# danini/multi-h

Measured on AMD Instinct MI355X. Metric: scored homography hypotheses/sec (50k pts x 100k models), higher is better.
Workload: dtype f64

## Files before the change

multi-h_amd/csrc/capi_engine.hpp:

```cpp
#pragma once
#include "../../include/multih_hip.h"
#include "mh_kernels.hpp"

#include <algorithm>
#include <chrono>
#include <cstdlib>
#include <cmath>
#include <cstdio>
#include <cstring>
#include <string>
#include <utility>
#include <atomic>
#include <memory>
#include <thread>
#include <vector>

using namespace mh;

extern thread_local std::string g_err;

inline int fail(int code, const std::string& msg)
{
    g_err = msg;
    return code;
// ... 168 lines not shown
    DevBuf<unsigned long long> sel_keys;
    int t_rank = 0, t_world = 1;
    mh_allgather_stream_fn t_stream_fn = nullptr;
    mh_allgather_dev_fn t_host_fn = nullptr;
    void* t_ctx = nullptr;
    Stream side_stream;
    Event ev_main, ev_side_pre;
    int tune_score32_resident = 12;
    int occ_score32 = -1, occ_cost32 = -1;
    int tune_cost32_batched = 0;
    int tune_cost32_slice_major = 0;
    int tune_sweep_slices = 0;
    int tune_dlt_variant = 0;
    int tune_cost32_resident = 8;
    int tune_stream_shift = 0;
    Stream dummy_streams[16];
    int tune_dlt_first = 1;
    static constexpr int PF_DEPTH = 2;
    DevBuf<double> pf_H[PF_DEPTH];
    DevBuf<int> pf_samples[PF_DEPTH];
    int pf_m[PF_DEPTH] = { 0, 0 };
    Event pf_ev[PF_DEPTH];
    int pf_head = 0, pf_count = 0;
    Stream xchg_stream;
    Event ev_sweep, ev_x[3];
    CountsSlot counts_waiting[2];
    long long xchg_calls = 0;
    long long models_seq = 0, best_models_seq = -1;
    bool counts_zeroed = false;
    bool counts_fresh = false;
    bool xchg_pending = false;
    PinnedBuf<int> h_best;
    int best_seq = 0;
    PinnedBuf<int> h_sel;
    long long copies_h2d = 0, copies_d2h = 0;

    int fm = 0;
    int fund_metric = 0;
    DevBuf<double> fund, fund_one;
    DevBuf<int> fund_samples, fund_counts, fund_inl;
    int fund_tuple = 8;
    int f7_m = 0;
    DevBuf<int> fund_nvalid, fund_stop;
    DevBuf<unsigned char> fund_mask, ref_keep, ref_in, ref_reason;
    int ref_reason_n = 0;
    DevBuf<double> ref_out;

    DevBuf<double> loc_H, loc_feat, ms_data, ms_mean;
    DevBuf<int> ms_votes, ms_out, ms_list, ms_pcnt, ms_heads, ms_tickets;
    DevBuf<double> ms_partial, ms_partial2;
    DevBuf<unsigned long long> ms_ticks;
    DevBuf<int> ms_ctl, ms_pcnt2;
    int ms_persist_per_cu = -1, ms_persist_per_cu6 = -1;
    int tune_select_refine = 0;
    int estimator = MH_ESTIMATOR_HAF;
    int data_term = MH_DATA_TERM_REFERENCE;
    DevBuf<int> r3_scratch;
    int tune_3pt_form = 0;
    DevBuf<double> sel_refit;
    DevBuf<int> sel_refit_ctr;
    DevBuf<double> ms_rs;
    DevBuf<int> ms_order, ms_cells, ms_cursor, ms_cellcount;
    int tune_ms_indexed = 1;
    int tune_ms_dense = 8;
    long long ms_indexed_launches = 0;
    int tune_ms_persist = 12;
    long long ms_persist_launches = 0, ms_persist_fallbacks = 0, ms_rounds = 0;

    int cost_L = 0;
    DevBuf<int> cost, labels_in, labels_pts, label_counts;
    DevBuf<int> ew_label, ew_cur, ew_trace, ew_saved, d_order, d_wsum;
    int comp_moves = 0;
    DevBuf<int> ew_comp, ew_comp_out;
    int trace_moves = 0;
    int detail_move = -1;
    ExpandCtxBufs ew_ctx[EXPAND_MAX_CTX];
    DevBuf<int> ew_bctl;
    PinnedBuf<int> h_batch;
    int tune_expand_ctx = 16;
    int tune_batch_min_labels = 16;
    int tune_batch_spw = 0;
    int cu_count = 256;
    DevBuf<int> sweep_ctl;
    int sweep_wg_per_cu = -1;
    int tune_sweep_headroom = 0;
    int solve_grid_max = 0;
    double longest_barrier_wait_ms = 0.0;
    int last_expand_retries = 0;
    long long expand_retries_total = 0;
    int last_solve_grid = 0;
    int inject_select_failure = 0;
    int inject_barrier_timeouts = 0;
    int inject_solve_failure = 0;
    PinnedBuf<int> h_flags;
    PinnedBuf<long long> h_acc;
    PinnedBuf<MeanShiftResultBlock> h_ms;
    PinnedBuf<int> h_ms_list;
    DevBuf<double> sel_pts[4];
    DevBuf<int> sel_pack_count;
    DevBuf<double> sel_gone[4];
    int tune_select_decrement = 1;
    int tune_knn_grid = 1;
    DevBuf<int> knn_cell, knn_count, knn_start, knn_orig;
    DevBuf<float> knn_P;
    DevBuf<int> knn_tmp, knn_part_i;
    DevBuf<float> knn_part_d;
    int sampler = MH_SAMPLER_UNIFORM, sampler_uniform_per_16 = 0;
    DevBuf<int> smp_nbr;
    int smp_k = 0;
    Dlt4Local dlt_local() const { return sampler == MH_SAMPLER_LOCAL ? Dlt4Local{ smp_nbr.p, smp_k, sampler_uniform_per_16 } : Dlt4Local{}; }

    bool profiling = false;
    KernelTimer timers[MH_K_COUNT_];
    int tune_residual_variant = 0;
    int tune_ld = 0;
    int tune_score_variant = 0;
    int residual_mode = MH_RESIDUAL_FORWARD;
    int tune_ms_batch = 6;
    int tune_reduce = 2;
    int tune_reduce_launches = 1;
    int tune_recycle = 1;
    int tune_expand[4] = { 128, 512, 1, 256 };
    int tune_cascade_iters = 2;
    int tune_push_mult = 6;
    ExpandStats last_expand{};

    double bbox[4] = { NAN, NAN, NAN, NAN };
    bool coords32_ok = false;
    double absmax_x = NAN, absmax_y = NAN, absmax_dst = NAN;
    int tune_score32_tiling = 0;
    int tune_score32 = 1;
    DevBuf<float> H32;
    DevBuf<unsigned long long> fb_pairs;
    long long score_pairs = 0;
    long long score_pairs_plain_fp64 = 0;
    DevBuf<int> weights, weights_counts;
    long long weights_models_seq = -1;
    PinnedBuf<int> h_best_w;
    Points pts() const { return Points{ x1.p, y1.p, x2.p, y2.p, n, bbox[0], bbox[1], bbox[2], bbox[3] }; }
};

namespace mhe {

template <typename Fn>
int guarded(Fn&& fn)
{
    try {
        return fn();
    } catch (const std::bad_alloc&) {
        return fail(MH_ERR_INVALID, "out of host memory");
    } catch (const std::exception& ex) {
        return fail(MH_ERR_INVALID, std::string("internal error: ") + ex.what());
    } catch (...) {
        return fail(MH_ERR_INVALID, "internal error");
    }
}

struct ScopedTimer {
    mh_engine* e;
    int k;
    hipStream_t st;
    Event a, b;
    bool on = false;
    ScopedTimer(mh_engine* e_, int k_, hipStream_t on_stream = nullptr) : e(e_), k(k_), st(on_stream ? on_stream : e_->stream)
    {
        if (!e->profiling || a.ensure(hipEventDefault) != hipSuccess || b.ensure(hipEventDefault) != hipSuccess) return;
        (void)hipEventRecord(a, st);
// ... 56 lines not shown
```

multi-h_amd/csrc/capi_score.hip:

```cpp
#include "capi_engine.hpp"

namespace mhe {

static bool pretest_usable(const mh_engine* e, double thr2, bool plain_variant_only)
{
    if (plain_variant_only && e->tune_score_variant != 0) return false;
    return e->tune_score32 && e->coords32_ok && thr2 >= 0x1p-40 && thr2 <= 0x1p40;
}

static int ensure_sweep_ctl(mh_engine* e)
{
    if (!e->sweep_ctl.p) {
        HIPCHK(e->sweep_ctl.reserve(2));
        HIPCHK(hipMemsetAsync(e->sweep_ctl.p, 0, sizeof(int) * 2, e->stream));
    }
    return MH_OK;
}

int score_models(mh_engine* e, const Points& p, const double* Hs, int m, double thr2, const unsigned char* dmask, int* counts_dev)
{
    const bool fwd = e->residual_mode != MH_RESIDUAL_SYMMETRIC;
    if (fwd && m > 0 && pretest_usable(e, thr2, true)) {
        HIPCHK(e->H32.reserve((size_t)m * 16));
        HIPCHK(e->fb_pairs.reserve(1));
// ... 147 lines not shown
    return guarded([&]() -> int {
    if (!e) return fail(MH_ERR_INVALID, "null engine");
    if (mode != MH_RESIDUAL_FORWARD && mode != MH_RESIDUAL_SYMMETRIC) return fail(MH_ERR_INVALID, "unknown residual mode");
    e->residual_mode = mode;
    return MH_OK;
    });
}

int mh_score(mh_engine* e, double thr2, const unsigned char* point_mask, int* counts)
{
    return guarded([&]() -> int {
    bool empty_shard = false;
    int rc = require_models_or_empty_shard(e, &empty_shard);
    if (rc || empty_shard) return rc;
    HIPCHK(reserve_counts(e, (size_t)e->m + 1));
    const unsigned char* dmask = nullptr;
    if (point_mask) {
        HIPCHK(e->mask.reserve((size_t)e->n + 2));
        HIPCHK(hipMemcpyAsync(e->mask.p, point_mask, e->n, hipMemcpyHostToDevice, e->stream));
        dmask = e->mask.p;
    }
    {
        ScopedTimer t(e, MH_K_SCORE);
        rc = score_models(e, e->pts(), e->H.p, e->m, thr2, dmask, e->counts.p);
        if (rc) return rc;
    }
    counts_scored(e);
    if (counts) {
        HIPCHK(hipMemcpyAsync(counts, e->counts.p, sizeof(int) * e->m, hipMemcpyDeviceToHost, e->stream));
        HIPCHK(hipStreamSynchronize(e->stream));
    }
    return MH_OK;
    });
}

int mh_score_msac(mh_engine* e, double thr2, const unsigned char* point_mask, int* counts, int* weights)
{
    return guarded([&]() -> int {
    bool empty_shard = false;
    int rc = require_models_or_empty_shard(e, &empty_shard);
    if (rc || empty_shard) return rc;
    if (e->residual_mode == MH_RESIDUAL_SYMMETRIC) return fail(MH_ERR_INVALID, "mh_score_msac: forward residual only");
    if ((long long)e->n * MH_MSAC_SCALE > 2147483647ll) return fail(MH_ERR_OVERFLOW, "mh_score_msac: n * MH_MSAC_SCALE exceeds int32");
    HIPCHK(reserve_counts(e, (size_t)e->m + 1));
    HIPCHK(e->weights.reserve((size_t)e->m + 1));
    HIPCHK(e->weights_counts.reserve((size_t)e->m + 1));
    const unsigned char* dmask = nullptr;
    if (point_mask) {
        HIPCHK(e->mask.reserve((size_t)e->n + 2));
        HIPCHK(hipMemcpyAsync(e->mask.p, point_mask, e->n, hipMemcpyHostToDevice, e->stream));
        dmask = e->mask.p;
    }
    e->weights_models_seq = -1;
    {
        ScopedTimer t(e, MH_K_SCORE);
        rc = msac_models(e, e->pts(), e->H.p, e->m, thr2, dmask, e->counts.p, e->weights.p, false);
        if (rc) return rc;
    }
    HIPCHK(hipMemcpyAsync(e->weights_counts.p, e->counts.p, sizeof(int) * (size_t)e->m, hipMemcpyDeviceToDevice, e->stream));
    counts_scored(e);
    e->weights_models_seq = e->models_seq;
    if (counts) HIPCHK(hipMemcpyAsync(counts, e->counts.p, sizeof(int) * e->m, hipMemcpyDeviceToHost, e->stream));
    if (weights) HIPCHK(hipMemcpyAsync(weights, e->weights.p, sizeof(int) * e->m, hipMemcpyDeviceToHost, e->stream));
    if (counts || weights) HIPCHK(hipStreamSynchronize(e->stream));
    return MH_OK;
    });
}

int mh_residual_matrix(mh_engine* e, double thr2, double* R_host, int* counts)
{
    return guarded([&]() -> int {
    bool empty_shard = false;
    int rc = require_models_or_empty_shard(e, &empty_shard);
    if (rc || empty_shard) return rc;
    e->ldr = residual_ld(e->n);
    size_t r_elems = (size_t)e->m * (size_t)e->ldr;
#ifdef MH_TUNING
    if (e->tune_ld > 0) { e->ldr = std::max<long long>(e->tune_ld, e->ldr); r_elems = (size_t)e->m * (size_t)e->ldr; }
    r_elems = std::max(r_elems, (size_t)((e->m + 15) / 16 * 16) * (size_t)((e->n + 1023) / 1024 * 1024));
#endif
    HIPCHK(e->R.reserve(r_elems));
    HIPCHK(reserve_counts(e, (size_t)e->m + 1));
    int resident = 0;
    if (e->tune_sweep_headroom >= 0 && e->residual_mode != MH_RESIDUAL_SYMMETRIC && (e->tune_residual_variant == 0 || (e->tune_residual_variant >= 50 && e->tune_residual_variant <= 52))) {
        if (e->sweep_wg_per_cu < 0) e->sweep_wg_per_cu = residual_workgroups_per_cu();
        const int headroom = e->tune_sweep_headroom > 0 ? e->tune_sweep_headroom : (e->t_stream_fn && e->t_world > 1 ? 32 : 0);
        resident = e->sweep_wg_per_cu * e->cu_count - headroom;
        if (resident < e->cu_count) resident = 0;
        if (resident > 0) {
            rc = ensure_sweep_ctl(e);
            if (rc) return rc;
        }
    }
    if (e->pf_count == 1 && e->tune_dlt_first && e->ev_side_pre) HIPCHK(hipStreamWaitEvent(e->stream, e->ev_side_pre, 0));
    {
        ScopedTimer t(e, MH_K_RESIDUAL);
        SweepLaunch how;
        how.slices = e->tune_sweep_slices;
        how.slice_major = e->tune_sweep_slices > 0 ? 1 : 0;
        how.counts_zeroed = e->counts_zeroed;
        how.resident_grid = resident;
        how.resident_ctl = e->sweep_ctl.p;
        HIPCHK(launch_residual(e->pts(), e->H.p, e->m, thr2, e->R.p, e->ldr, e->counts.p,
                               e->residual_mode == MH_RESIDUAL_SYMMETRIC ? -1 : e->tune_residual_variant, e->stream, how));
    }
    counts_scored(e);
    if (R_host)
        HIPCHK(hipMemcpy2DAsync(R_host, sizeof(double) * e->n, e->R.p, sizeof(double) * e->ldr,
                                sizeof(double) * e->n, e->m, hipMemcpyDeviceToHost, e->stream));
    if (counts)
        HIPCHK(hipMemcpyAsync(counts, e->counts.p, sizeof(int) * e->m, hipMemcpyDeviceToHost, e->stream));
    if (R_host || counts) HIPCHK(hipStreamSynchronize(e->stream));
    return MH_OK;
    });
}

int mh_cost_matrix(mh_engine* e, int* C_host, int* counts)
{
    return guarded([&]() -> int {
    bool empty_shard = false;
    int rc = require_models_or_empty_shard(e, &empty_shard);
    if (rc || empty_shard) return rc;
    e->ldc = cost_ld(e->n);
    HIPCHK(e->C.reserve((size_t)e->m * (size_t)e->ldc));
    HIPCHK(reserve_counts(e, (size_t)e->m + 1));
    {
        ScopedTimer t(e, MH_K_COSTMATRIX);
        const double thr2 = e->thr_H * e->thr_H;
        if (pretest_usable(e, thr2, false)) {
            HIPCHK(e->H32.reserve((size_t)e->m * 16));
            HIPCHK(launch_model32(e->H.p, e->m, e->absmax_x, e->absmax_y, e->absmax_dst, e->H32.p, e->stream));
            int* ctl = nullptr;
            if (e->tune_cost32_resident != 0) {
                rc = ensure_sweep_ctl(e);
                if (rc) return rc;
                ctl = e->sweep_ctl.p;
            }
            HIPCHK(launch_cost32(e->pts(), e->H.p, e->H32.p, e->m, e->lambda, thr2, e->absmax_dst, e->C.p, e->ldc, e->counts.p, e->stream,
                                 ctl, e->cu_count, e->tune_cost32_resident > 0 ? e->tune_cost32_resident : 0, e->tune_cost32_slice_major, e->tune_cost32_batched, &e->occ_cost32,
                                 e->data_term == MH_DATA_TERM_RISING));
        } else
            HIPCHK(launch_cost_matrix(e->pts(), e->H.p, e->m, e->lambda, thr2, e->C.p, e->ldc, e->counts.p, e->stream,
                                      e->data_term == MH_DATA_TERM_RISING));
    }
    counts_scored(e);
    if (C_host)
        HIPCHK(hipMemcpy2DAsync(C_host, sizeof(int) * e->n, e->C.p, sizeof(int) * e->ldc, sizeof(int) * e->n, e->m,
                                hipMemcpyDeviceToHost, e->stream));
    if (counts) HIPCHK(hipMemcpyAsync(counts, e->counts.p, sizeof(int) * e->m, hipMemcpyDeviceToHost, e->stream));
    if (C_host || counts) HIPCHK(hipStreamSynchronize(e->stream));
    return MH_OK;
    });
}

int mh_get_residual_rows(mh_engine* e, int first, int count, double* rows_host)
{
    return guarded([&]() -> int {
    int rc = require_models(e);
    if (rc) return rc;
    if (!e->R.p || e->ldr <= 0) return fail(MH_ERR_NOT_SET, "residual matrix has not been computed");
    if (first < 0 || count <= 0 || first + count > e->m || !rows_host)
        return fail(MH_ERR_INVALID, "row range out of bounds or null output");
    HIPCHK(hipMemcpy2DAsync(rows_host, sizeof(double) * e->n, e->R.p + (size_t)first * e->ldr,
                            sizeof(double) * e->ldr, sizeof(double) * e->n, count,
                            hipMemcpyDeviceToHost, e->stream));
    HIPCHK(hipStreamSynchronize(e->stream));
    return MH_OK;
    });
}

int mh_prefetch_dlt4(mh_engine* e, unsigned long long seed, long long first, int m)
{
    return guarded([&]() -> int {
    int rc = require_points(e);
    if (rc) return rc;
    if (m <= 0) return fail(MH_ERR_INVALID, "m must be positive");
    if (e->n < 4) return fail(MH_ERR_INVALID, "need at least 4 correspondences");
    if (e->sampler == MH_SAMPLER_LOCAL && e->smp_k <= 0) return fail(MH_ERR_NOT_SET, "the local sampler has no table; call mh_build_sample_neighbours");
    rc = ensure_side_stream(e);
    if (rc) return rc;
    if (e->pf_count >= mh_engine::PF_DEPTH) return fail(MH_ERR_INVALID, "two batches are already prefetched: adopt one first (mh_adopt_prefetched)");
    const int slot = (e->pf_head + e->pf_count) % mh_engine::PF_DEPTH;
    if (e->pf_H[slot].cap < (size_t)m * 9 || e->pf_samples[slot].cap < (size_t)m * 4) {
        HIPCHK(hipStreamSynchronize(e->side_stream));
        HIPCHK(hipStreamSynchronize(e->stream));
        HIPCHK(e->pf_H[slot].reserve((size_t)m * 9));
        HIPCHK(e->pf_samples[slot].reserve((size_t)m * 4));
// ... 111 lines not shown
```

multi-h_amd/csrc/mh_kernels.hpp:

```cpp
#pragma once
#include <hip/hip_runtime.h>
#include <cstdint>

namespace mh {

struct Points {
    const double* x1;
    const double* y1;
    const double* x2;
    const double* y2;
    int n;
    double xmin, xmax, ymin, ymax;
};

struct Affines {
    const double* a11;
    const double* a12;
    const double* a21;
    const double* a22;
};

struct Epipolar {
    double F[9];
    double ex, ey;
};

inline long long residual_ld(int n) { return ((long long)n + 15) & ~15ll; }

struct SweepLaunch {
    int slices = 0;
    bool contiguous = false;
    int swapxy = 0;
    bool counts_zeroed = false;
    int resident_grid = 0;
    int* resident_ctl = nullptr;
    int slice_major = 0;
};
hipError_t launch_residual(const Points& p, const double* H, int M, double thr2, double* R,
                           long long ldr, int* counts, int variant, hipStream_t s, const SweepLaunch& how);
int residual_workgroups_per_cu();
hipError_t launch_score(const Points& p, const double* H, int M, double thr2,
                        const unsigned char* mask, int* counts, int variant, hipStream_t s);
hipError_t launch_model32(const double* H, int M, double X, double Y, double Cmax, float* H32 , hipStream_t s);
hipError_t launch_score32(const Points& p, const double* H, const float* H32, int M, double thr2, double Cmax, const unsigned char* mask,
                          int* counts, unsigned long long* fallback_pairs, int tiling, hipStream_t s, int* resident_ctl = nullptr,
                          int cu_count = 256, int resident_slices = 0, int* occ_cache = nullptr);
hipError_t launch_cost32(const Points& p, const double* H, const float* H32, int M, double lambda, double thr2, double Cmax,
                         int* C, long long ldc, int* counts, hipStream_t s, int* resident_ctl = nullptr, int cu_count = 256,
                         int psplit_override = 0, int slice_major = 0, int batched = 0, int* occ_cache = nullptr, int rising = 0);
hipError_t launch_msac32(const Points& p, const double* H, const float* H32, int M, double thr2, double Cmax, const unsigned char* mask,
                         int* counts, int* weights, unsigned long long* fp64_pairs, hipStream_t s);
hipError_t launch_msac64(const Points& p, const double* H, int M, double thr2, const unsigned char* mask, int* counts, int* weights,
                         hipStream_t s);
hipError_t launch_inliers_of_model(const Points& p, const double* H, int idx, double thr2,
                                   int label_value, int* labels, hipStream_t s);
hipError_t launch_moments(const Points& p, const double* H, int M, double thr2, double* moments,
                          double* min_eig, hipStream_t s);

hipError_t launch_compat_select(const double* pts , const int* begin , int clusters,
                                const int* tri , const double* H ,
                                const unsigned char* ok, int trials, double* out , hipStream_t s);
hipError_t launch_compat_fit(const double* pts, const int* begin, int clusters, const int* tri, const double F[9], int trials,
                             double* H, unsigned char* ok, hipStream_t s);

struct Dlt4Local { const int* nbr = nullptr; int k = 0; int uniform_per_16 = 0; };
hipError_t launch_dlt4(const Points& p, unsigned long long seed, long long first, int M,
                       int* idx_out, double* H_out, hipStream_t s, int variant = 0 ,
                       Dlt4Local local = Dlt4Local{});

hipError_t launch_fund8(const Points& p, unsigned long long seed, long long first, int M,
                        int* idx_out , double* F_out, hipStream_t s);

hipError_t launch_fund7(const Points& p, unsigned long long seed, long long first, int M,
                        int* idx_out , double* F_out , int* nvalid_out , hipStream_t s);

hipError_t launch_ransac_stop(const int* counts , const int* nvalid , int S, int n, double confidence,
                              const double* F , double* F_win, int* out, hipStream_t s);
hipError_t launch_fund_mask(const Points& p, const double* F_in, double thr2, unsigned char* mask_out, int* count,
                            hipStream_t s, int metric);
hipError_t launch_sampson_score(const Points& p, const double* F, int M, double thr2, int* counts,
                                hipStream_t s, int metric);
hipError_t launch_fund_refit(const Points& p, const double* F_in, double thr2, double* F_out,
                             unsigned char* mask_out, int* count_out, hipStream_t s, int metric);

constexpr int REFIT_H_MAX_ITERATIONS = 16;
hipError_t launch_refit_h(const Points& p, const double* H_in, double thr2, int iterations, double* H_out,
                          unsigned char* mask_out, int* out_i, hipStream_t s);

inline long long cost_ld(int n) { return ((long long)n + 31) & ~31ll; }
hipError_t launch_cost_matrix(const Points& p, const double* H, int M, double lambda, double thr2, int* C, long long ldc,
                              int* counts, hipStream_t s, int rising = 0);
hipError_t launch_data_cost(const Points& p, const double* H, int Nh, double lambda, double thr2,
                            int* cost, hipStream_t s, int rising = 0);

hipError_t launch_reestimate(const Points& p, const Affines& a, const int* labels, int Nh,
                             const Epipolar& ep, double* H, int* counts, hipStream_t s);

size_t reestimate_3pt_scratch_ints(int n, int Nh);
hipError_t launch_reestimate_3pt(const Points& p, const int* labels, int Nh, const Epipolar& ep, double* H, int* counts,
                                 int* scratch, hipStream_t s, int form = 0);

hipError_t launch_haf_point(const Points& p, const Affines& a, const Epipolar& ep, double locality,
                            double* H_out , double* feat_out ,
                            hipStream_t s);

hipError_t launch_haf_propose(const Points& p, const Affines& a, const Epipolar& ep, const int* nbr, int k, int members,
                              double thr2, long long first, int m, int stride, double* H_out, unsigned* used_out, hipStream_t s);

hipError_t launch_propose_3pt(const Points& p, const double F[9], unsigned long long seed, long long first, int M,
                              int* idx_out, double* H_out, hipStream_t s, Dlt4Local local = Dlt4Local{});

hipError_t launch_refine_points(const Points& p, const Affines& a, const double F[9], const double e1[2],
                                const double e2[2], const unsigned char* in_mask, unsigned char* keep,
                                double* out , unsigned char* reason , hipStream_t s,
                                int points_only = 0);

constexpr int MS_BATCH = 256;
struct MeanShiftWork {
    const double* data;
    int n, d;
    double* mean;
    int* votes;
    int* out;
// ... 185 lines not shown
```

multi-h_amd/csrc/residual.hip:

```cpp

#include <type_traits>

#include "mh_kernels.hpp"
#include "mh_device.hpp"

namespace mh {

typedef double __attribute__((address_space(1))) gdouble;
typedef char __attribute__((address_space(1))) gchar;

namespace cfg {
struct Base {
    static constexpr bool WRITE_R = false, MASK = false, SYM = false, NT = false, FAST = true, HSGPR = false, LEAN = false, SEMI = true;
    static constexpr bool CALIB = false, CONTRACT = false, TILED = false;
    static constexpr int SF = 0, MINW = 1;
};
struct Sweep : Base { static constexpr int PPL = 4, MC = 64; static constexpr bool WRITE_R = true, NT = true, HSGPR = true, LEAN = true; };
struct SweepSym : Base { static constexpr int PPL = 4, MC = 16; static constexpr bool WRITE_R = true, NT = true, HSGPR = true, SYM = true; };
struct Score : Base { static constexpr int PPL = 4, MC = 16; static constexpr bool HSGPR = true, LEAN = true; };
struct ScoreMasked : Score { static constexpr bool MASK = true; };
struct ScoreSym : Base { static constexpr int PPL = 4, MC = 16; static constexpr bool SYM = true; };
struct ScoreSymMasked : ScoreSym { static constexpr bool MASK = true; };
template <class... C> constexpr bool no_measurement_switch = ((!C::CALIB && !C::CONTRACT && !C::TILED && C::SF == 0 && C::MINW == 1 && C::FAST && C::PPL == 4) && ...);
static_assert(no_measurement_switch<Sweep, SweepSym, Score, ScoreMasked, ScoreSym, ScoreSymMasked>, "a measurement switch in a product form");
}
using ProductSweep = cfg::Sweep;

template <class Cfg> constexpr bool on_resident_grid = false;
template <> constexpr bool on_resident_grid<ProductSweep> = true;

template <class Cfg>
__device__ __forceinline__ void
residual_wg(const double* __restrict__ x1, const double* __restrict__ y1,
            const double* __restrict__ x2, const double* __restrict__ y2, int N,
            const double* __restrict__ H, int M, double thr2, double* __restrict__ R,
            long long ldr, int* __restrict__ counts, const unsigned char* __restrict__ mask,
            int psplit, double bx0, double bx1, double by0, double by1, const int bx, const int by)
{
    constexpr int PPL = Cfg::PPL, MC = Cfg::MC, SF = Cfg::SF;
    constexpr bool WRITE_R = Cfg::WRITE_R, MASK = Cfg::MASK, NT = Cfg::NT, FAST = Cfg::FAST, CALIB = Cfg::CALIB, HSGPR = Cfg::HSGPR,
                   SYM = Cfg::SYM, CONTRACT = Cfg::CONTRACT, LEAN = Cfg::LEAN, TILED = Cfg::TILED, SEMI = Cfg::SEMI;
    constexpr int CH = PPL / 2;
    constexpr int WAVE_PTS = 64 * PPL;
    constexpr int TILE = 4 * WAVE_PTS;
    const int lane = threadIdx.x & 63;
    const int wave = __builtin_amdgcn_readfirstlane(threadIdx.x >> 6);
    const int m0 = bx * MC;

    __shared__ double s_h[MC * 9];
    __shared__ double s_a[SYM ? MC * 9 : 1];
    for (int i = threadIdx.x; i < MC * 9; i += 256) {
        const size_t g = (size_t)m0 * 9 + i;
        s_h[i] = (g < (size_t)M * 9) ? H[g] : 0.0;
    }
    __shared__ int s_hok[MC];
    __shared__ int s_far[MC];
    __shared__ int s_aok[SYM ? MC : 1];
    __syncthreads();
    if (threadIdx.x < MC) {
        const double* h = s_h + 9 * threadIdx.x;
        s_hok[threadIdx.x] = model_pre(h);
        s_far[threadIdx.x] = model_far(h, bx0, bx1, by0, by1);
        if (SYM) {
            double* a = s_a + 9 * threadIdx.x;
            a[0] = h[4] * h[8] - h[5] * h[7]; a[1] = h[2] * h[7] - h[1] * h[8]; a[2] = h[1] * h[5] - h[2] * h[4];
            a[3] = h[5] * h[6] - h[3] * h[8]; a[4] = h[0] * h[8] - h[2] * h[6]; a[5] = h[2] * h[3] - h[0] * h[5];
            a[6] = h[3] * h[7] - h[4] * h[6]; a[7] = h[1] * h[6] - h[0] * h[7]; a[8] = h[0] * h[4] - h[1] * h[3];
            s_aok[threadIdx.x] = model_pre(a);
        }
    }
    __syncthreads();

    const unsigned long long hok_bits = __builtin_amdgcn_ballot_w64(lane < MC && s_hok[lane < MC ? lane : 0] != 0);
    const unsigned long long far_bits = __builtin_amdgcn_ballot_w64(lane < MC && s_far[lane < MC ? lane : 0] != 0);

    unsigned lane_bytes = (unsigned)lane * 16u;

    int cnt = 0;
    static_assert(MC <= 64, "one counting lane per model");

    const int nslices = psplit > 0 ? psplit : -psplit;
    const int ntiles_all = (N + TILE - 1) / TILE;
    const int per_slice = (ntiles_all + nslices - 1) / nslices;
    const int base0 = psplit > 0 ? by * TILE : by * per_slice * TILE;
    const int base_end = psplit > 0 ? N : min(N, (by + 1) * per_slice * TILE);
    const int base_step = psplit > 0 ? psplit * TILE : TILE;
    for (int base = base0; base < base_end; base += base_step) {
        double px[PPL], py[PPL], qx[PPL], qy[PPL];
        bool ok[PPL], pok[PPL], pokb[SYM ? PPL : 1];
        unsigned long long okm[PPL];
        const int wbase = base + wave * WAVE_PTS;
#pragma unroll
        for (int c = 0; c < CH; ++c) {
            const int n = wbase + c * 128 + lane * 2;
            if (n + 1 < N) {
                const double2 a = *reinterpret_cast<const double2*>(x1 + n);
                const double2 b = *reinterpret_cast<const double2*>(y1 + n);
                const double2 cc = *reinterpret_cast<const double2*>(x2 + n);
                const double2 d = *reinterpret_cast<const double2*>(y2 + n);
                px[2 * c] = a.x; px[2 * c + 1] = a.y;
                py[2 * c] = b.x; py[2 * c + 1] = b.y;
                qx[2 * c] = cc.x; qx[2 * c + 1] = cc.y;
                qy[2 * c] = d.x; qy[2 * c + 1] = d.y;
                ok[2 * c] = true; ok[2 * c + 1] = true;
            } else if (n < N) {
                px[2 * c] = x1[n]; py[2 * c] = y1[n]; qx[2 * c] = x2[n]; qy[2 * c] = y2[n];
                px[2 * c + 1] = 1.0; py[2 * c + 1] = 1.0; qx[2 * c + 1] = 1.0; qy[2 * c + 1] = 1.0;
                ok[2 * c] = true; ok[2 * c + 1] = false;
            } else {
                px[2 * c] = 1.0; py[2 * c] = 1.0; qx[2 * c] = 1.0; qy[2 * c] = 1.0;
                px[2 * c + 1] = 1.0; py[2 * c + 1] = 1.0; qx[2 * c + 1] = 1.0; qy[2 * c + 1] = 1.0;
                ok[2 * c] = false; ok[2 * c + 1] = false;
            }
            if (MASK) {
                if (ok[2 * c]) ok[2 * c] = mask[n] != 0;
                if (ok[2 * c + 1]) ok[2 * c + 1] = mask[n + 1] != 0;
            }
            okm[2 * c] = __builtin_amdgcn_ballot_w64(ok[2 * c]);
            okm[2 * c + 1] = __builtin_amdgcn_ballot_w64(ok[2 * c + 1]);
            pok[2 * c] = point_pre(px[2 * c], py[2 * c], qx[2 * c], qy[2 * c]);
            pok[2 * c + 1] = point_pre(px[2 * c + 1], py[2 * c + 1], qx[2 * c + 1], qy[2 * c + 1]);
            if (SYM) {
                pokb[2 * c] = point_pre(qx[2 * c], qy[2 * c], px[2 * c], py[2 * c]);
                pokb[2 * c + 1] = point_pre(qx[2 * c + 1], qy[2 * c + 1], px[2 * c + 1], py[2 * c + 1]);
            }
        }

        bool tile_lean = false;
        if (LEAN) {
            bool lane_ok = true;
#pragma unroll
            for (int q = 0; q < PPL; ++q) lane_ok = lane_ok && ok[q] && pok[q];
            tile_lean = (wbase + WAVE_PTS <= N) && (__builtin_amdgcn_ballot_w64(lane_ok) == ~0ull);
        }
        const int tile_idx = base / TILE;

#pragma unroll 1
        for (int mi = 0; mi < MC; ++mi) {
            const int m = m0 + mi;
            if (m < M) {
                const double* h = HSGPR ? (H + 9 * (size_t)m) : (s_h + 9 * mi);
                const double h0 = h[0], h1 = h[1], h2 = h[2], h3 = h[3], h4 = h[4], h5 = h[5],
                             h6 = h[6], h7 = h[7], h8 = h[8];
                const bool hok = ((hok_bits >> mi) & 1ull) != 0;
                const bool far = FAST && !CONTRACT && ((far_bits >> mi) & 1ull) != 0;
                const bool aok = SYM ? (s_aok[mi] != 0) : false;
                int c_m = 0;
                auto row_ptr = [&](int n) -> double* {
                    if (TILED) return R + ((size_t)bx * ntiles_all + tile_idx) * ((size_t)MC * TILE) + (size_t)mi * TILE + (n - base);
                    return R + (size_t)m * ldr + n;
                };
                gchar* row_base = (gchar*)row_ptr(wbase);
                asm volatile("" : "+v"(lane_bytes));
                asm volatile("" : "+s"(row_base));
                auto sweep = [&](auto schk) {
                    constexpr bool SCHK = decltype(schk)::value;
#pragma unroll
                    for (int c = 0; c < CH; ++c) {
                        if (CALIB) {
                            const int n = wbase + c * 128 + lane * 2;
                            if (n + 1 < N)
                                *reinterpret_cast<double2*>(R + (size_t)m * ldr + n) =
                                    make_double2(px[2 * c] + h0, py[2 * c] + h0);
                            continue;
                        }
                        double d0s, d1s;
                        const double d0 = CONTRACT ? fwd_d2_contracted(h0, h1, h2, h3, h4, h5, h6, h7, h8, px[2 * c],
                                                                       py[2 * c], qx[2 * c], qy[2 * c])
                                          : FAST ? fwd_d2_fast<SCHK>(h0, h1, h2, h3, h4, h5, h6, h7, h8, px[2 * c],
                                                                   py[2 * c], qx[2 * c], qy[2 * c], pok[2 * c] && hok)
                                               : fwd_d2(h0, h1, h2, h3, h4, h5, h6, h7, h8, px[2 * c],
                                                        py[2 * c], qx[2 * c], qy[2 * c]);
                        const double d1 = CONTRACT ? fwd_d2_contracted(h0, h1, h2, h3, h4, h5, h6, h7, h8, px[2 * c + 1],
                                                                       py[2 * c + 1], qx[2 * c + 1], qy[2 * c + 1])
                                          : FAST ? fwd_d2_fast<SCHK>(h0, h1, h2, h3, h4, h5, h6, h7, h8, px[2 * c + 1],
                                                                   py[2 * c + 1], qx[2 * c + 1], qy[2 * c + 1], pok[2 * c + 1] && hok)
                                               : fwd_d2(h0, h1, h2, h3, h4, h5, h6, h7, h8, px[2 * c + 1],
                                                        py[2 * c + 1], qx[2 * c + 1], qy[2 * c + 1]);
                        d0s = d0; d1s = d1;
                        if (SYM) {
                            const double* a = s_a + 9 * mi;
                            const double b0 = fwd_d2_fast<true>(a[0], a[1], a[2], a[3], a[4], a[5], a[6], a[7], a[8],
                                                                qx[2 * c], qy[2 * c], px[2 * c], py[2 * c], pokb[2 * c] && aok);
                            const double b1 = fwd_d2_fast<true>(a[0], a[1], a[2], a[3], a[4], a[5], a[6], a[7], a[8],
                                                                qx[2 * c + 1], qy[2 * c + 1], px[2 * c + 1], py[2 * c + 1],
                                                                pokb[2 * c + 1] && aok);
                            d0s = d0 + b0;
                            d1s = d1 + b1;
                        }
                        if (WRITE_R) {
                            const int n = wbase + c * 128 + lane * 2;
                            gdouble* dstp = reinterpret_cast<gdouble*>(row_base + lane_bytes) + c * 128;
                            if (n + 1 < N) {
                                if (NT) {
                                    __builtin_nontemporal_store(d0s, dstp);
                                    __builtin_nontemporal_store(d1s, dstp + 1);
                                } else {
                                    dstp[0] = d0s; dstp[1] = d1s;
                                }
                            } else if (n < N) {
                                dstp[0] = d0s;
                            }
                        }
                        c_m += __builtin_popcountll(__builtin_amdgcn_ballot_w64(d0s < thr2) & okm[2 * c]);
                        c_m += __builtin_popcountll(__builtin_amdgcn_ballot_w64(d1s < thr2) & okm[2 * c + 1]);
                    }
                };
                bool lean_done = false;
                if (LEAN && FAST && !SYM && !CONTRACT && !CALIB && tile_lean && hok && (SEMI || far)) {
                    double dl[PPL], sq[PPL];
                    unsigned long long bad = 0ull;
#pragma unroll
                    for (int q = 0; q < PPL; ++q)
                        dl[q] = fwd_d2_lean(h0, h1, h2, h3, h4, h5, h6, h7, h8, px[q], py[q], qx[q], qy[q], sq[q]);
                    if (!far) {
#pragma unroll
                        for (int q = 0; q < PPL; ++q) bad |= __builtin_amdgcn_ballot_w64(!(__builtin_fabs(sq[q]) >= 0x1p-255));
                    }
                    if (bad == 0ull) {
                        lean_done = true;
#pragma unroll
                        for (int c = 0; c < CH; ++c) {
                            const double d0 = dl[2 * c], d1 = dl[2 * c + 1];
                            if (WRITE_R) {
                                gdouble* dstp = reinterpret_cast<gdouble*>(row_base + lane_bytes) + c * 128;
                                if (SF != 0) {
                                    typedef double d2v __attribute__((ext_vector_type(2)));
                                    const d2v val = { d0, d1 };
                                    if (SF == 2) asm volatile("global_store_dwordx4 %0, %1, off sc1" :: "v"(dstp), "v"(val) : "memory");
                                    else if (SF == 3) asm volatile("global_store_dwordx4 %0, %1, off sc0 sc1" :: "v"(dstp), "v"(val) : "memory");
                                    else if (SF == 4) asm volatile("global_store_dwordx4 %0, %1, off sc1 nt" :: "v"(dstp), "v"(val) : "memory");
                                    else asm volatile("global_store_dwordx4 %0, %1, off sc0 sc1 nt" :: "v"(dstp), "v"(val) : "memory");
                                } else if (NT) {
                                    __builtin_nontemporal_store(d0, dstp);
                                    __builtin_nontemporal_store(d1, dstp + 1);
                                } else {
                                    dstp[0] = d0; dstp[1] = d1;
                                }
                            }
                            c_m += __builtin_popcountll(__builtin_amdgcn_ballot_w64(d0 < thr2));
                            c_m += __builtin_popcountll(__builtin_amdgcn_ballot_w64(d1 < thr2));
                        }
                    }
                }
                if (lean_done) {}
                else if (far) sweep(std::false_type{});
                else sweep(std::true_type{});
                const int c_new = __builtin_amdgcn_readlane(cnt, mi) + c_m;
                asm("s_mov_b32 m0, %2\n\ts_nop 0\n\tv_writelane_b32 %0, %1, m0" : "+v"(cnt) : "s"(c_new), "s"(mi) : "m0");
            }
        }
    }

    __shared__ int s_cnt[4][MC];
    if (lane < MC) s_cnt[wave][lane] = cnt;
    __syncthreads();
    if (threadIdx.x < MC && m0 + (int)threadIdx.x < M) {
        const int t = threadIdx.x;
        const int c = s_cnt[0][t] + s_cnt[1][t] + s_cnt[2][t] + s_cnt[3][t];
        if (nslices == 1) counts[m0 + t] = c;
        else atomicAdd(&counts[m0 + t], c);
    }
}

template <class Cfg>
__global__ void __launch_bounds__(256, Cfg::MINW)
k_residual(const double* __restrict__ x1, const double* __restrict__ y1,
           const double* __restrict__ x2, const double* __restrict__ y2, int N,
           const double* __restrict__ H, int M, double thr2, double* __restrict__ R,
           long long ldr, int* __restrict__ counts, const unsigned char* __restrict__ mask,
           int psplit, int swapxy, double bx0, double bx1, double by0, double by1)
{
    const int bx = swapxy ? blockIdx.y : blockIdx.x;
    const int by = swapxy ? blockIdx.x : blockIdx.y;
    residual_wg<Cfg>(x1, y1, x2, y2, N, H, M, thr2, R, ldr, counts, mask, psplit, bx0, bx1, by0, by1, bx, by);
}

template <class Cfg>
__global__ void __launch_bounds__(256, Cfg::MINW) __attribute__((amdgpu_num_vgpr(88)))
k_residual_resident(const double* __restrict__ x1, const double* __restrict__ y1,
                    const double* __restrict__ x2, const double* __restrict__ y2, int N,
                    const double* __restrict__ H, int M, double thr2, double* __restrict__ R,
                    long long ldr, int* __restrict__ counts, const unsigned char* __restrict__ mask,
                    int psplit, int gx, int nitems, int* __restrict__ ctl, double bx0, double bx1, double by0, double by1, int slice_major)
{
    __shared__ int s_item;
#pragma unroll 1
    for (;;) {
        if (threadIdx.x == 0) s_item = atomicAdd(&ctl[0], 1);
        __syncthreads();
        const int item = s_item;
        if (item >= nitems) break;
        int bx, by;
        if (slice_major) { bx = item / psplit; by = item - bx * psplit; }
        else { by = item / gx; bx = item - by * gx; }
        residual_wg<Cfg>(x1, y1, x2, y2, N, H, M, thr2, R, ldr, counts, mask, psplit, bx0, bx1, by0, by1, bx, by);
        __syncthreads();
    }
    if (threadIdx.x == 0 && atomicAdd(&ctl[1], 1) == (int)gridDim.x - 1) {
        ctl[1] = 0;
        __hip_atomic_store(&ctl[0], 0, __ATOMIC_RELEASE, __HIP_MEMORY_SCOPE_AGENT);
    }
}

template <class Cfg>
static hipError_t launch_rs(const Points& p, const double* H, int M, double thr2, double* R,
                            long long ldr, int* counts, const unsigned char* mask, hipStream_t s, const SweepLaunch& how = {})
{
    constexpr int PPL = Cfg::PPL, MC = Cfg::MC;
    if (M <= 0 || p.n <= 0) return hipSuccess;
    const int gx = (M + MC - 1) / MC;
    const int tile = 256 * PPL;
    const int ntiles = (p.n + tile - 1) / tile;
    int psplit = 1;
    if (Cfg::WRITE_R) {
        psplit = (37500 + gx - 1) / gx;
        if (psplit < 4 && ntiles >= 32) psplit = 4;
        if (psplit > ntiles) psplit = ntiles;
        if (psplit < 1) psplit = 1;
    } else if (gx < 1024) {
        psplit = (2048 + gx - 1) / gx;
        if (psplit > ntiles) psplit = ntiles;
        if (psplit < 1) psplit = 1;
    } else if (ntiles >= 32) {
        psplit = 4;
    }
    const bool forced = how.slices > 0, contiguous = forced && how.contiguous;
    if (forced) psplit = how.slices < ntiles ? how.slices : ntiles;
    if (psplit > 1 && !how.counts_zeroed) {
        hipError_t e = hipMemsetAsync(counts, 0, sizeof(int) * (size_t)M, s);
        if (e != hipSuccess) return e;
    }
    if constexpr (on_resident_grid<Cfg>)
    if (how.resident_grid > 0 && how.resident_ctl && !contiguous && !how.swapxy && gx * psplit > how.resident_grid) {
        hipLaunchKernelGGL(k_residual_resident<Cfg>, dim3(how.resident_grid), dim3(256), 0, s, p.x1, p.y1, p.x2, p.y2, p.n, H, M, thr2, R,
                           ldr, counts, mask, psplit, gx, gx * psplit, how.resident_ctl, p.xmin, p.xmax, p.ymin, p.ymax, how.slice_major);
        return hipGetLastError();
    }
    dim3 grid(gx, psplit);
    if (how.swapxy) grid = dim3(psplit, gx);
    hipLaunchKernelGGL(k_residual<Cfg>, grid, dim3(256), 0, s, p.x1, p.y1, p.x2, p.y2, p.n, H, M, thr2, R, ldr, counts, mask,
                       contiguous ? -psplit : psplit, how.swapxy, p.xmin, p.xmax, p.ymin, p.ymax);
    return hipGetLastError();
}

#ifdef MH_TUNING
namespace tune {
static hipError_t launch_residual_variant(const Points& p, const double* H, int M, double thr2, double* R, long long ldr, int* counts,
                                          int variant, hipStream_t s, const SweepLaunch& how);
static hipError_t launch_score_variant(const Points& p, const double* H, int M, double thr2, int* counts, int variant, hipStream_t s);
}
#endif

hipError_t launch_residual(const Points& p, const double* H, int M, double thr2, double* R,
                           long long ldr, int* counts, int variant, hipStream_t s, const SweepLaunch& how)
{
    auto run = [&](auto form, const SweepLaunch& o = {}) { return launch_rs<decltype(form)>(p, H, M, thr2, R, ldr, counts, nullptr, s, o); };
    if (variant == 0) return run(ProductSweep{}, how);
    if (variant == -1) return run(cfg::SweepSym{});
#ifdef MH_TUNING
    return tune::launch_residual_variant(p, H, M, thr2, R, ldr, counts, variant, s, how);
#else
    return hipErrorInvalidValue;
#endif
}

int residual_workgroups_per_cu()
{
    int n = 0;
    const hipError_t he = hipOccupancyMaxActiveBlocksPerMultiprocessor(&n, (const void*)k_residual_resident<ProductSweep>, 256, 0);
    return he == hipSuccess && n > 0 ? n : 0;
}

hipError_t launch_score(const Points& p, const double* H, int M, double thr2,
                        const unsigned char* mask, int* counts, int variant, hipStream_t s)
{
    auto run = [&](auto form) { return launch_rs<decltype(form)>(p, H, M, thr2, nullptr, 0, counts, mask, s); };
    if (variant == -1) return mask ? run(cfg::ScoreSymMasked{}) : run(cfg::ScoreSym{});
    if (mask) return run(cfg::ScoreMasked{});
    if (variant == 0) return run(cfg::Score{});
#ifdef MH_TUNING
    return tune::launch_score_variant(p, H, M, thr2, counts, variant, s);
#else
    return hipErrorInvalidValue;
#endif
}

#ifdef MH_TUNING
#include "residual_variants.hpp"
#endif

__global__ void __launch_bounds__(256)
k_inliers_of_model(const double* __restrict__ x1, const double* __restrict__ y1,
                   const double* __restrict__ x2, const double* __restrict__ y2, int N,
                   const double* __restrict__ H, int idx, double thr2, int label_value,
                   int* __restrict__ labels)
{
    const int n = blockIdx.x * 256 + threadIdx.x;
    if (n >= N) return;
    const double* h = H + 9 * (size_t)idx;
    const double d2 = fwd_d2(h[0], h[1], h[2], h[3], h[4], h[5], h[6], h[7], h[8], x1[n], y1[n],
                             x2[n], y2[n]);
    if (d2 < thr2) labels[n] = label_value;
}

hipError_t launch_inliers_of_model(const Points& p, const double* H, int idx, double thr2,
                                   int label_value, int* labels, hipStream_t s)
{
    hipLaunchKernelGGL(k_inliers_of_model, dim3((p.n + 255) / 256), dim3(256), 0, s, p.x1, p.y1,
                       p.x2, p.y2, p.n, H, idx, thr2, label_value, labels);
    return hipGetLastError();
}

__global__ void __launch_bounds__(256)
k_moments(const double* __restrict__ x1, const double* __restrict__ y1,
          const double* __restrict__ x2, const double* __restrict__ y2, int N,
          const double* __restrict__ H, double thr2, double* __restrict__ moments,
          double* __restrict__ min_eig)
{
    const int m = blockIdx.x;
    const int t = threadIdx.x;
    const double* h = H + 9 * (size_t)m;
    const double h0 = h[0], h1 = h[1], h2 = h[2], h3 = h[3], h4 = h[4], h5 = h[5], h6 = h[6],
                 h7 = h[7], h8 = h[8];
    double acc[5] = { 0.0, 0.0, 0.0, 0.0, 0.0 };
    int cnt = 0;
    constexpr int UNROLL = 8;
    for (int n0 = t; n0 < N; n0 += 256 * UNROLL) {
        double px[UNROLL], py[UNROLL], qx[UNROLL], qy[UNROLL];
#pragma unroll
        for (int j = 0; j < UNROLL; ++j) {
            const int n = n0 + 256 * j, mm = n < N ? n : 0;
            px[j] = x1[mm]; py[j] = y1[mm]; qx[j] = x2[mm]; qy[j] = y2[mm];
        }
#pragma unroll
        for (int j = 0; j < UNROLL; ++j) {
            if (n0 + 256 * j >= N) continue;
            const double x = px[j], y = py[j];
            const double d2 = fwd_d2(h0, h1, h2, h3, h4, h5, h6, h7, h8, x, y, qx[j], qy[j]);
            if (d2 < thr2) {
                acc[0] = acc[0] + x;
                acc[1] = acc[1] + y;
                acc[2] = acc[2] + x * x;
                acc[3] = acc[3] + x * y;
                acc[4] = acc[4] + y * y;
                ++cnt;
            }
        }
    }
    __shared__ double sv[256][5];
    __shared__ int sc[256];
#pragma unroll
    for (int k = 0; k < 5; ++k) sv[t][k] = acc[k];
// ... 39 lines not shown
```

Before: 13.39 million.

## Give symmetric residual forms the lean fast path, wider model tiles and resident grid

Symmetric residual and score forms now use the lean fast path, adding the backward transfer distance inline when the inverse is valid. The symmetric sweep also gets a 64-model tile and a persistent resident-grid kernel with its own cached occupancy. The aim is to cut per-point branching and launch/tail overhead in symmetric mode. The metric is probably forward scoring, which this may not touch, and the larger tile at a 128-VGPR cap risks spills.

Result: slower. 13.24 million (-1.1%).

```diff
diff --git a/multi-h_amd/csrc/capi_engine.hpp b/multi-h_amd/csrc/capi_engine.hpp
--- a/multi-h_amd/csrc/capi_engine.hpp
+++ b/multi-h_amd/csrc/capi_engine.hpp
@@ -274,7 +274,7 @@
     int tune_batch_spw = 0;
     int cu_count = 256;
     DevBuf<int> sweep_ctl;
-    int sweep_wg_per_cu = -1;
+    int sweep_wg_per_cu[2] = { -1, -1 };
     int tune_sweep_headroom = 0;
     int solve_grid_max = 0;
     double longest_barrier_wait_ms = 0.0;
diff --git a/multi-h_amd/csrc/capi_score.hip b/multi-h_amd/csrc/capi_score.hip
--- a/multi-h_amd/csrc/capi_score.hip
+++ b/multi-h_amd/csrc/capi_score.hip
@@ -253,10 +253,12 @@
     HIPCHK(e->R.reserve(r_elems));
     HIPCHK(reserve_counts(e, (size_t)e->m + 1));
     int resident = 0;
-    if (e->tune_sweep_headroom >= 0 && e->residual_mode != MH_RESIDUAL_SYMMETRIC && (e->tune_residual_variant == 0 || (e->tune_residual_variant >= 50 && e->tune_residual_variant <= 52))) {
-        if (e->sweep_wg_per_cu < 0) e->sweep_wg_per_cu = residual_workgroups_per_cu();
+    const bool sym = e->residual_mode == MH_RESIDUAL_SYMMETRIC;
+    if (e->tune_sweep_headroom >= 0 && (sym || e->tune_residual_variant == 0 || (e->tune_residual_variant >= 50 && e->tune_residual_variant <= 52))) {
+        int& wg_per_cu = e->sweep_wg_per_cu[sym ? 1 : 0];
+        if (wg_per_cu < 0) wg_per_cu = residual_workgroups_per_cu(sym);
         const int headroom = e->tune_sweep_headroom > 0 ? e->tune_sweep_headroom : (e->t_stream_fn && e->t_world > 1 ? 32 : 0);
-        resident = e->sweep_wg_per_cu * e->cu_count - headroom;
+        resident = wg_per_cu * e->cu_count - headroom;
         if (resident < e->cu_count) resident = 0;
         if (resident > 0) {
             rc = ensure_sweep_ctl(e);
@@ -273,7 +275,7 @@
         how.resident_grid = resident;
         how.resident_ctl = e->sweep_ctl.p;
         HIPCHK(launch_residual(e->pts(), e->H.p, e->m, thr2, e->R.p, e->ldr, e->counts.p,
-                               e->residual_mode == MH_RESIDUAL_SYMMETRIC ? -1 : e->tune_residual_variant, e->stream, how));
+                               sym ? -1 : e->tune_residual_variant, e->stream, how));
     }
     counts_scored(e);
     if (R_host)
diff --git a/multi-h_amd/csrc/mh_kernels.hpp b/multi-h_amd/csrc/mh_kernels.hpp
--- a/multi-h_amd/csrc/mh_kernels.hpp
+++ b/multi-h_amd/csrc/mh_kernels.hpp
@@ -38,7 +38,7 @@
 };
 hipError_t launch_residual(const Points& p, const double* H, int M, double thr2, double* R,
                            long long ldr, int* counts, int variant, hipStream_t s, const SweepLaunch& how);
-int residual_workgroups_per_cu();
+int residual_workgroups_per_cu(bool symmetric);
 hipError_t launch_score(const Points& p, const double* H, int M, double thr2,
                         const unsigned char* mask, int* counts, int variant, hipStream_t s);
 hipError_t launch_model32(const double* H, int M, double X, double Y, double Cmax, float* H32 , hipStream_t s);
diff --git a/multi-h_amd/csrc/residual.hip b/multi-h_amd/csrc/residual.hip
--- a/multi-h_amd/csrc/residual.hip
+++ b/multi-h_amd/csrc/residual.hip
@@ -16,18 +16,20 @@
     static constexpr int SF = 0, MINW = 1;
 };
 struct Sweep : Base { static constexpr int PPL = 4, MC = 64; static constexpr bool WRITE_R = true, NT = true, HSGPR = true, LEAN = true; };
-struct SweepSym : Base { static constexpr int PPL = 4, MC = 16; static constexpr bool WRITE_R = true, NT = true, HSGPR = true, SYM = true; };
+struct SweepSym : Base { static constexpr int PPL = 4, MC = 64; static constexpr bool WRITE_R = true, NT = true, HSGPR = true, SYM = true, LEAN = true; };
 struct Score : Base { static constexpr int PPL = 4, MC = 16; static constexpr bool HSGPR = true, LEAN = true; };
 struct ScoreMasked : Score { static constexpr bool MASK = true; };
-struct ScoreSym : Base { static constexpr int PPL = 4, MC = 16; static constexpr bool SYM = true; };
+struct ScoreSym : Base { static constexpr int PPL = 4, MC = 16; static constexpr bool SYM = true, HSGPR = true, LEAN = true; };
 struct ScoreSymMasked : ScoreSym { static constexpr bool MASK = true; };
 template <class... C> constexpr bool no_measurement_switch = ((!C::CALIB && !C::CONTRACT && !C::TILED && C::SF == 0 && C::MINW == 1 && C::FAST && C::PPL == 4) && ...);
 static_assert(no_measurement_switch<Sweep, SweepSym, Score, ScoreMasked, ScoreSym, ScoreSymMasked>, "a measurement switch in a product form");
+static_assert(SweepSym::LEAN && ScoreSym::LEAN && ScoreSymMasked::LEAN && ScoreSym::HSGPR && ScoreSymMasked::HSGPR, "the symmetric forms share one body");
 }
 using ProductSweep = cfg::Sweep;
 
 template <class Cfg> constexpr bool on_resident_grid = false;
 template <> constexpr bool on_resident_grid<ProductSweep> = true;
+template <> constexpr bool on_resident_grid<cfg::SweepSym> = true;
 
 template <class Cfg>
 __device__ __forceinline__ void
@@ -130,7 +132,7 @@
         if (LEAN) {
             bool lane_ok = true;
 #pragma unroll
-            for (int q = 0; q < PPL; ++q) lane_ok = lane_ok && ok[q] && pok[q];
+            for (int q = 0; q < PPL; ++q) lane_ok = lane_ok && ok[q] && pok[q] && (!SYM || pokb[SYM ? q : 0]);
             tile_lean = (wbase + WAVE_PTS <= N) && (__builtin_amdgcn_ballot_w64(lane_ok) == ~0ull);
         }
         const int tile_idx = base / TILE;
@@ -145,6 +147,7 @@
                 const bool hok = ((hok_bits >> mi) & 1ull) != 0;
                 const bool far = FAST && !CONTRACT && ((far_bits >> mi) & 1ull) != 0;
                 const bool aok = SYM ? (s_aok[mi] != 0) : false;
+                const double* am = s_a + 9 * mi;
                 int c_m = 0;
                 auto row_ptr = [&](int n) -> double* {
                     if (TILED) return R + ((size_t)bx * ntiles_all + tile_idx) * ((size_t)MC * TILE) + (size_t)mi * TILE + (n - base);
@@ -179,7 +182,7 @@
                                                         py[2 * c + 1], qx[2 * c + 1], qy[2 * c + 1]);
                         d0s = d0; d1s = d1;
                         if (SYM) {
-                            const double* a = s_a + 9 * mi;
+                            const double* a = am;
                             const double b0 = fwd_d2_fast<true>(a[0], a[1], a[2], a[3], a[4], a[5], a[6], a[7], a[8],
                                                                 qx[2 * c], qy[2 * c], px[2 * c], py[2 * c], pokb[2 * c] && aok);
                             const double b1 = fwd_d2_fast<true>(a[0], a[1], a[2], a[3], a[4], a[5], a[6], a[7], a[8],
@@ -207,13 +210,22 @@
                     }
                 };
                 bool lean_done = false;
-                if (LEAN && FAST && !SYM && !CONTRACT && !CALIB && tile_lean && hok && (SEMI || far)) {
+                if (LEAN && FAST && !CONTRACT && !CALIB && tile_lean && hok && (SEMI || far) && (!SYM || aok)) {
                     double dl[PPL], sq[PPL];
                     unsigned long long bad = 0ull;
 #pragma unroll
                     for (int q = 0; q < PPL; ++q)
                         dl[q] = fwd_d2_lean(h0, h1, h2, h3, h4, h5, h6, h7, h8, px[q], py[q], qx[q], qy[q], sq[q]);
                     if (!far) {
+#pragma unroll
+                        for (int q = 0; q < PPL; ++q) bad |= __builtin_amdgcn_ballot_w64(!(__builtin_fabs(sq[q]) >= 0x1p-255));
+                    }
+                    if constexpr (SYM) {
+                        const double a0 = am[0], a1 = am[1], a2 = am[2], a3 = am[3], a4 = am[4], a5 = am[5],
+                                     a6 = am[6], a7 = am[7], a8 = am[8];
+#pragma unroll
+                        for (int q = 0; q < PPL; ++q)
+                            dl[q] = dl[q] + fwd_d2_lean(a0, a1, a2, a3, a4, a5, a6, a7, a8, qx[q], qy[q], px[q], py[q], sq[q]);
 #pragma unroll
                         for (int q = 0; q < PPL; ++q) bad |= __builtin_amdgcn_ballot_w64(!(__builtin_fabs(sq[q]) >= 0x1p-255));
                     }
@@ -304,6 +316,34 @@
 }
 
 template <class Cfg>
+__global__ void __launch_bounds__(256, Cfg::MINW) __attribute__((amdgpu_num_vgpr(128)))
+k_symmetric_resident(const double* __restrict__ x1, const double* __restrict__ y1,
+                     const double* __restrict__ x2, const double* __restrict__ y2, int N,
+                     const double* __restrict__ H, int M, double thr2, double* __restrict__ R,
+                     long long ldr, int* __restrict__ counts, const unsigned char* __restrict__ mask,
+                     int psplit, int gx, int nitems, int* __restrict__ ctl, double bx0, double bx1, double by0, double by1, int slice_major)
+{
+    static_assert(Cfg::SYM, "the forward forms run in k_residual_resident");
+    __shared__ int s_item;
+#pragma unroll 1
+    for (;;) {
+        if (threadIdx.x == 0) s_item = atomicAdd(&ctl[0], 1);
+        __syncthreads();
+        const int item = s_item;
+        if (item >= nitems) break;
+        int bx, by;
+        if (slice_major) { bx = item / psplit; by = item - bx * psplit; }
+        else { by = item / gx; bx = item - by * gx; }
+        residual_wg<Cfg>(x1, y1, x2, y2, N, H, M, thr2, R, ldr, counts, mask, psplit, bx0, bx1, by0, by1, bx, by);
+        __syncthreads();
+    }
+    if (threadIdx.x == 0 && atomicAdd(&ctl[1], 1) == (int)gridDim.x - 1) {
+        ctl[1] = 0;
+        __hip_atomic_store(&ctl[0], 0, __ATOMIC_RELEASE, __HIP_MEMORY_SCOPE_AGENT);
+    }
+}
+
+template <class Cfg>
 static hipError_t launch_rs(const Points& p, const double* H, int M, double thr2, double* R,
                             long long ldr, int* counts, const unsigned char* mask, hipStream_t s, const SweepLaunch& how = {})
 {
@@ -333,6 +373,10 @@
     }
     if constexpr (on_resident_grid<Cfg>)
     if (how.resident_grid > 0 && how.resident_ctl && !contiguous && !how.swapxy && gx * psplit > how.resident_grid) {
+        if constexpr (Cfg::SYM)
+            hipLaunchKernelGGL(k_symmetric_resident<Cfg>, dim3(how.resident_grid), dim3(256), 0, s, p.x1, p.y1, p.x2, p.y2, p.n, H, M, thr2, R,
+                               ldr, counts, mask, psplit, gx, gx * psplit, how.resident_ctl, p.xmin, p.xmax, p.ymin, p.ymax, how.slice_major);
+        else
         hipLaunchKernelGGL(k_residual_resident<Cfg>, dim3(how.resident_grid), dim3(256), 0, s, p.x1, p.y1, p.x2, p.y2, p.n, H, M, thr2, R,
                            ldr, counts, mask, psplit, gx, gx * psplit, how.resident_ctl, p.xmin, p.xmax, p.ymin, p.ymax, how.slice_major);
         return hipGetLastError();
@@ -357,7 +401,7 @@
 {
     auto run = [&](auto form, const SweepLaunch& o = {}) { return launch_rs<decltype(form)>(p, H, M, thr2, R, ldr, counts, nullptr, s, o); };
     if (variant == 0) return run(ProductSweep{}, how);
-    if (variant == -1) return run(cfg::SweepSym{});
+    if (variant == -1) return run(cfg::SweepSym{}, how);
 #ifdef MH_TUNING
     return tune::launch_residual_variant(p, H, M, thr2, R, ldr, counts, variant, s, how);
 #else
@@ -365,10 +409,11 @@
 #endif
 }
 
-int residual_workgroups_per_cu()
+int residual_workgroups_per_cu(bool symmetric)
 {
     int n = 0;
-    const hipError_t he = hipOccupancyMaxActiveBlocksPerMultiprocessor(&n, (const void*)k_residual_resident<ProductSweep>, 256, 0);
+    const void* kernel = symmetric ? (const void*)k_symmetric_resident<cfg::SweepSym> : (const void*)k_residual_resident<ProductSweep>;
+    const hipError_t he = hipOccupancyMaxActiveBlocksPerMultiprocessor(&n, kernel, 256, 0);
     return he == hipSuccess && n > 0 ? n : 0;
 }
 
```
